# indrajeetadityaroy9/vit-inductive-bias-distillation

Hardware: AMD Instinct MI355X
Metric: distillation images/sec (BASD loss fwd+bwd+grad all-reduce), DeiT-S<-ResNet-50 @ bs256/GPU (higher is better)
Workload: dtype f32; 1 GPU; cfg2 DeiT-S<-ResNet-50 224x224; per_gpu_batch=256, global_batch=256, input_dtype=float32, layout=strided (CLS-sliced / channel-major views), backward=True, grad_allreduce_bytes=88202672, grad_allreduce=none at world size 1 (bucket packed, nothing to exchange), rank_readback=auto, readback_deferred_steps=1756, selector=basd_selector_chain mode 0, parallelism=dp1

## Files before the change

include/basd_hip.h:

```cpp
#ifndef BASD_HIP_H
#define BASD_HIP_H

#include <stdint.h>

#ifdef __cplusplus
extern "C" {
#endif

#ifndef __HIP_PLATFORM_AMD__
typedef struct ihipStream_t* hipStream_t;
#endif

#define BASD_OK 0
#define BASD_EINVAL (-1)
#define BASD_EUNSUPPORTED (-2)
#define BASD_DTYPE_F32 0
#define BASD_DTYPE_BF16 1
#define BASD_DTYPE_U8 2


int basd_gemm_nt(const void* a, int a_dtype, long a_sb, long a_sn, long a_sd, int a_rows_per_batch,
                 long a_batch_stride, const float* b, long ldb, long b_batch_stride, int M, int N, int K, int batch,
                 float* c, long ldc, long c_batch_stride, float scale, const float* bias, float beta,
                 float* colsum_part, float* col_mean, hipStream_t stream);
// ... 8 lines not shown
int basd_colmean_parts(int rows);

int basd_colmean(const void* x, int dtype, long sb, long sn, long sd, int rows_per_batch, long batch_stride,
                 int rows, int cols, int batch, int parts, float* partial, float* mean, hipStream_t stream);

int basd_gemm_tuning(int split_bf16);
int basd_gemm_tuning_get(void);

int basd_colmean_multi(const void* const* x_ptrs, int dtype, long sb, long sn, long sd, int rows_per_batch, int rows,
                       int cols, int n_mats, int parts, float* partial, float* means, int vec_ok,
                       hipStream_t stream);

int basd_syrk_splits(int krows, int cols, int n_mats);

int basd_syrk_multi(const void* const* x_ptrs, int dtype, long sb, long sn, long sd, int rows_per_batch, int krows,
                    int cols, int n_mats, const float* means, const float* scales, int splits, float* slabs,
                    float* out, long out_stride, int vec_ok, const float* fold, int fold_parts, int fold_from,
                    hipStream_t stream);


int basd_jacobi_workspace_ints(int batch, int max_sweeps);
int basd_jacobi_max_rows(void);
int basd_jacobi_plain4_fits(int n);

int basd_jacobi_tuning(int lanes_per_pair);
int basd_jacobi_ordering(int odd_even);

int basd_jacobi_onesided(float* W, long batch_stride, int rows_dot, int rows_tot, int n, int batch,
                         const int* n_arr, float* colnorm, int colnorm_stride, int max_sweeps, float tol_cos,
                         int* flags, int* sweeps_out, hipStream_t stream);

long basd_jacobi_twopass_workspace_bytes(int n, int batch, int max_sweeps);
int basd_jacobi_stacked_twopass(float* W, long batch_stride, int n, int batch, float* colnorm, int colnorm_stride,
                                int max_sweeps, float tol_cos, void* workspace, int* sweeps_out, hipStream_t stream);

int basd_sort_extract(const float* W, long batch_stride, int rows, int rows_tot, int n, int batch,
                      const float* colnorm, int colnorm_stride, float* vals_desc, float* vecs, int kmax,
                      hipStream_t stream);


long basd_tridiag_workspace_bytes(int n, int batch);

int basd_tridiag(float* a, long a_batch_stride, int n, int batch, float* d, float* e, float* tau, float* vh,
                 void* work, hipStream_t stream);

int basd_tridiag_ranked(float* a, long a_batch_stride, int n, int batch, float* d, float* e, float* tau, float* vh,
                        void* work, int rank_count, double factor, int cap, int* rank_out, int* host_mirror,
                        void* mid_event ,
                        hipStream_t stream);

int basd_tridiag_tuning(int members, int pad, int lag, int threads, int tail, int reset);

int basd_tridiag_eigenvalues(const float* d, const float* e, int n, int batch, float* vals_desc, hipStream_t stream);

int basd_tridiag_apply_q(const float* tau, const float* vh, int n, int k, int batch, const float* x, float* out,
                         int k_stride, int transpose, hipStream_t stream);

int basd_tridiag_shifted_solve(const float* d, const float* e, const float* shifts, int shift_stride, int n, int k,
                               int batch, const float* rhs, float* x, hipStream_t stream);

int basd_tridiag_mp_rank(const float* d, const float* e, int n, int batch, double factor, int cap, int* rank_out,
                         float* thr_out, const int* status, int* host_mirror, hipStream_t stream);

int basd_tridiag_eigenvectors(const float* d, const float* e, const float* tau, const float* vh,
                              const float* vals_desc, int n, int k, int batch, float* z, float* vecs, int k_stride,
                              hipStream_t stream);


int basd_mp_rank(const float* vals_desc, int n, int batch, double factor, int cap, int* rank_out, float* thr_out,
                 hipStream_t stream);

int basd_grassmann_distance(const float* colnorm, int stride, const int* k_arr, const float* sw, int sw_stride,
                            const int* sw_index, int items, float* d_out, float* theta_out, hipStream_t stream);

int basd_grassmann_distance_padded(const float* colnorm, int stride, int n_valid, const int* k_arr, const float* sw,
                                   int sw_stride, const int* sw_index, int items, float* d_out, hipStream_t stream);

int basd_sqrt_clamp(const float* in, float* out, long count, hipStream_t stream);

int basd_gram_finish(const float* c, const float* zbar, int n, int batch, long m_rows, float* out_u, float* out_c,
                     hipStream_t stream);

int basd_selector_tail(const float* t_d, const float* t_e, const float* t_tau, const float* t_vh, const float* t_vals,
                       const float* s_d, const float* s_e, const float* s_tau, const float* s_vh, const float* s_vals,
                       int d_s, int E, int L, int kmax, const int* ranks, const float* proj_s_t, float* z_s,
                       float* v_s, float* z_t, float* u_t, float* u_rot, float* sw, float* cos, int* k_arr,
                       const int* sw_index, float* sigma, int* flags, float* d_out, hipStream_t stream);

int basd_tridiag_mp_rank_rank1(const float* d, const float* e, const float* w, int n, int batch, double rho,
                               double factor, int cap, int* rank_out, const int* status, int* host_mirror,
                               hipStream_t stream);

int basd_tridiag_ranked_gated(float* a, long a_batch_stride, int n, int batch, float* d, float* e, float* tau, float* vh,
                              void* work, int rank_count, double factor, int cap, int* rank_out, int* host_mirror,
                              const unsigned* go_flag, unsigned go_value, int go_budget, hipStream_t stream);
int basd_flag_set(unsigned* flag, unsigned value, hipStream_t stream);

typedef struct BasdSelectorChain {
    const void* const* teacher_host_ptrs;
    long t_dtype, t_sb, t_sn, t_sd;
    const void* const* student_ptrs;
    long s_dtype, s_sb, s_sn, s_sd, s_vec_ok;
    const float* proj_t;
    const float* proj_s_t;
    long E, L, B, n_s, n_t, d_s, d_t;
    double mp_factor;
// ... 326 lines not shown
```

vit-inductive-bias-distillation_amd/basd_amd/_lib.py:

```python
from __future__ import annotations

import ctypes as C
import os
import threading

_HERE = os.path.dirname(os.path.abspath(__file__))
LIB_PATH = os.path.join(_HERE, "libbasd_hip.so")

vp, i32, i64, f32, f64 = C.c_void_p, C.c_int, C.c_long, C.c_float, C.c_double

SIGNATURES = {
    "basd_gemm_nt": [vp, i32, i64, i64, i64, i32, i64, vp, i64, i64, i32, i32, i32, i32, vp, i64, i64, f32, vp, f32,
                     vp, vp, vp],
    "basd_gemm_tn_splits": [i32],
    "basd_gemm_tn": [vp, vp, i32, i64, i64, i64, i64, i64, i64, i64, i64, i32, i32, i32, i32, i32, vp, vp, i32, vp,
                     vp, i64, i64, f32, vp],
    "basd_colmean_parts": [i32],
    "basd_colmean": [vp, i32, i64, i64, i64, i32, i64, i32, i32, i32, i32, vp, vp, vp],
    "basd_colmean_multi": [vp, i32, i64, i64, i64, i32, i32, i32, i32, i32, vp, vp, i32, vp],
    "basd_syrk_splits": [i32, i32, i32],
    "basd_syrk_multi": [vp, i32, i64, i64, i64, i32, i32, i32, i32, vp, vp, i32, vp, vp, i64, i32, vp, i32, i32, vp],
    "basd_jacobi_workspace_ints": [i32, i32],
    "basd_jacobi_max_rows": [],
    "basd_jacobi_twopass_workspace_bytes": [i32, i32, i32],
    "basd_jacobi_stacked_twopass": [vp, i64, i32, i32, vp, i32, i32, f32, vp, vp, vp],
    "basd_jacobi_tuning": [i32],
    "basd_jacobi_ordering": [i32],
    "basd_gemm_tuning": [i32],
    "basd_gemm_tuning_get": [],
    "basd_jacobi_onesided": [vp, i64, i32, i32, i32, i32, vp, vp, i32, i32, f32, vp, vp, vp],
    "basd_sort_extract": [vp, i64, i32, i32, i32, i32, vp, i32, vp, vp, i32, vp],
    "basd_tridiag_workspace_bytes": [i32, i32],
    "basd_tridiag_tuning": [i32, i32, i32, i32, i32, i32],
    "basd_tridiag": [vp, i64, i32, i32, vp, vp, vp, vp, vp, vp],
    "basd_tridiag_ranked": [vp, i64, i32, i32, vp, vp, vp, vp, vp, i32, f64, i32, vp, vp, vp, vp],
    "basd_tridiag_ranked_gated": [vp, i64, i32, i32, vp, vp, vp, vp, vp, i32, f64, i32, vp, vp, vp, C.c_uint, i32, vp],
    "basd_flag_set": [vp, C.c_uint, vp],
    "basd_scale_unless_one": [vp, i64, vp, vp, vp],
    "basd_event_create": [vp],
    "basd_event_destroy": [vp],
    "basd_stream_wait_event": [vp, vp],
    "basd_tridiag_eigenvalues": [vp, vp, i32, i32, vp, vp],
    "basd_tridiag_apply_q": [vp, vp, i32, i32, i32, vp, vp, i32, i32, vp],
    "basd_tridiag_shifted_solve": [vp, vp, vp, i32, i32, i32, i32, vp, vp, vp],
    "basd_tridiag_mp_rank": [vp, vp, i32, i32, f64, i32, vp, vp, vp, vp, vp],
    "basd_tridiag_mp_rank_rank1": [vp, vp, vp, i32, i32, f64, f64, i32, vp, vp, vp, vp],
    "basd_tridiag_eigenvectors": [vp, vp, vp, vp, vp, i32, i32, i32, vp, vp, i32, vp],
    "basd_mp_rank": [vp, i32, i32, f64, i32, vp, vp, vp],
    "basd_grassmann_distance": [vp, i32, vp, vp, i32, vp, i32, vp, vp, vp],
    "basd_grassmann_distance_padded": [vp, i32, i32, vp, vp, i32, vp, i32, vp, vp],
    "basd_selector_tail": [vp] * 10 + [i32, i32, i32, i32] + [vp] * 14 + [vp],
    "basd_sqrt_clamp": [vp, vp, i64, vp],
    "basd_gram_finish": [vp, vp, i32, i32, i64, vp, vp, vp],
    "basd_cross_entropy": [vp, i32, i64, i32, i32, vp, vp, i64, f32, i64, vp, vp, vp],
    "basd_token_weights": [vp, i32, vp, i32, i64, i64, i64, i64, i32, i32, i32, i32, i32, i32, i32, vp, vp, vp, vp,
                           vp, vp, vp, vp, vp, vp],
    "basd_student_project": [vp, i32, i64, i64, i32, i32, i32, i32, vp, vp, vp, vp, vp, vp, vp, vp, vp, vp],
    "basd_teacher_center": [vp, i32, vp, i32, i64, i64, i64, i32, i32, i32, vp, vp, vp, vp, vp, vp, vp],
    "basd_teacher_center_multi": [vp, i32, vp, i32, i32, i64, i64, i64, i32, i32, i32, vp, vp, vp, vp, vp, vp, vp],
    "basd_teacher_center_stream_scratch_floats": [i32, i32, i32, i32],
    "basd_teacher_center_stream": [vp, i32, vp, i32, i32, i64, i64, i64, i32, i32, i32, vp, vp, vp, vp, vp, vp, vp, vp],
    "basd_gram_f64": [vp, i64, i32, i32, i32, vp, i64, vp],
    "basd_gram_f64_split": [vp, i64, i32, i32, i32, i32, vp, vp, vp],
    "basd_chol_f64": [vp, i64, i32, i32, vp, i64, vp],
    "basd_stack_product": [vp, vp, i64, i32, i32, i32, vp, i64, vp],
    "basd_procrustes_finalize": [vp, i64, vp, i32, i32, i32, i32, vp, i64, vp, vp, vp, vp, vp, i32, vp, vp, vp, vp,
                                 vp, vp],
    "basd_student_project_multi": [vp, i32, i64, i64, i32, i32, i32, i32, i32, i32, vp, i64, vp, vp, vp, vp, vp, vp,
                                   vp, vp, vp],
    "basd_student_grad_multi": [vp, i32, i64, i64, i32, i32, i32, i32, i32, vp, i64, vp, vp, vp, vp, vp, vp, f32, vp,
                                vp, vp, vp],
    "basd_student_grad_fused": [vp, i32, i64, i64, i32, i32, i32, i32, i32, i32, vp, i64, vp, vp, vp, vp, vp, vp, vp,
                                f32, vp, vp],
    "basd_procrustes_forward_fused": [vp, vp],
    "basd_procrustes_tuning": [i32],
    "basd_jacobi_plain4_fits": [i32],
    "basd_stack_product_t": [vp, vp, i64, i32, i32, i32, vp, i64, vp],
    "basd_kprime_from_transposed": [vp, i64, vp, i32, i32, vp, i64, i32, vp, i64, vp, vp],
    "basd_procrustes_finish_transposed": [vp, i64, vp, i32, i32, i32, i32, vp, i64, vp, vp, vp, vp, vp, i32, vp, vp, vp,
                                          vp, vp, i64, i32, vp, vp],
    "basd_procrustes_finish_tuning": [i32],
    "basd_ustack_stash": [vp, i64, i32, i32, vp, i64, vp],
    "basd_ustack_from_transposed": [vp, i64, vp, i32, i32, vp, i64, vp, i64, vp, i32, vp, vp],
    "basd_resample_tokens": [vp, i32, i64, i64, i64, i32, i32, i32, i32, vp, vp, vp, vp, vp],
    "basd_resample_tokens_adjoint": [vp, i32, i32, i32, i32, vp, vp, vp, vp, vp, vp, vp],
    "basd_teacher_factor": [vp, i64, vp, i32, i32, i32, vp, vp, i64, vp, vp, vp, vp, vp, vp, vp, vp, vp],
    "basd_teacher_factor_tiled": [vp, i64, vp, i32, i32, i32, vp, vp, i64, vp, vp, vp, vp, vp, vp, vp, vp, vp, vp],
    "basd_mix_grad_tokens": [vp, vp, i32, i32, i64, i64, i64, i32, i32, i32, i32, vp, vp, vp, vp, vp],
    "basd_mix_grad_tokens_scratch_floats": [i32, i32, i32, i32],
    "basd_mix_grad_tokens_onepass": [vp, vp, i32, i32, i64, i64, i64, i32, i32, i32, i32, vp, vp, vp, vp, vp, vp],
    "basd_token_weight_bwd": [vp, vp, i32, i32, i32, i32, vp, vp, vp, vp, vp, vp, i32, i32, i64, i64, i64, i64, i32,
                              i32, i32, vp, vp, vp],
    "basd_build_angle_stack": [vp, i32, vp, i32, vp, vp],
    "basd_grassmann_distance_bwd": [vp, vp, i32, vp, vp, i32, vp, vp, i32, vp, vp],
    "basd_eigvec_k2": [vp, vp, i32, i32, i32, vp, vp],
# ... 117 lines not shown
```

vit-inductive-bias-distillation_amd/csrc/chain.hip:

```cpp
#include "basd_common.h"
#include "../../include/basd_hip.h"
#include <stdlib.h>

namespace basd {

__global__ void __launch_bounds__(256) chain_sw_kernel(const float* __restrict__ vals, int n, int kmax,
                                                       float* __restrict__ sw) {
    const int l = blockIdx.x;
    for (int i = threadIdx.x; i < kmax; i += 256) sw[(long)l * kmax + i] = sqrtf(fmaxf(vals[(long)l * n + i], 0.f));
}

__global__ void chain_k_arr_kernel(const int* __restrict__ ranks, int L, int items, int kmax, int* __restrict__ k_arr) {
    const int i = blockIdx.x * blockDim.x + threadIdx.x;
    if (i < items) {
        int k = ranks[i % L];
        k = k < 1 ? 1 : k;
        k_arr[i] = k > kmax ? kmax : k;
    }
}

constexpr int CERT_BLOCKS = 32;
__global__ void __launch_bounds__(256) rank_certificate_kernel(const float* __restrict__ grams, const float* __restrict__ zbar,
                                                               int n, int L, double factor, double* __restrict__ scratch,
                                                               int* __restrict__ host_flag) {
// ... 90 lines not shown
    } while (0)
#define BASD_MARK(ev, stream)                                         \
    do {                                                              \
        if (ev) BASD_HIP(hipEventRecord((hipEvent_t)(ev), (stream))); \
    } while (0)

extern "C" {

int basd_event_record(void* ev, hipStream_t stream) {
    BASD_CHECK_ARG(ev);
    BASD_HIP(hipEventRecord((hipEvent_t)ev, stream));
    return BASD_OK;
}
int basd_event_synchronize(void* ev) {
    BASD_CHECK_ARG(ev);
    BASD_HIP(hipEventSynchronize((hipEvent_t)ev));
    return BASD_OK;
}
int basd_stream_create_priority(void** out, int level) {
    BASD_CHECK_ARG(out && level >= -1 && level <= 1);
    int least = 0, greatest = 0;
    BASD_HIP(hipDeviceGetStreamPriorityRange(&least, &greatest));
    const int prio = level < 0 ? greatest : (level > 0 ? least : 0);
    BASD_HIP(hipStreamCreateWithPriority((hipStream_t*)out, hipStreamNonBlocking, prio));
    return BASD_OK;
}

int basd_event_create_timed(void** out) {
    BASD_CHECK_ARG(out);
    BASD_HIP(hipEventCreateWithFlags((hipEvent_t*)out, hipEventDefault));
    return BASD_OK;
}
int basd_event_elapsed_ms(void* from, void* to, float* ms_out) {
    BASD_CHECK_ARG(from && to && ms_out);
    BASD_HIP(hipEventElapsedTime(ms_out, (hipEvent_t)from, (hipEvent_t)to));
    return BASD_OK;
}

int basd_selector_chain_tail(const BasdSelectorChain* a, int kmax, int exact_k) {
    BASD_CHECK_ARG(a && a->d && a->vals && a->zv && a->vecs && a->u_rot && a->sw && a->cos && a->sigma && a->d_out &&
                   a->k_arr && a->sw_index && a->jflags && a->ranks && a->proj_s_t);
    const int E = (int)a->E, L = (int)a->L, n = (int)a->d_s;
    BASD_CHECK_ARG(E > 0 && L > 0 && kmax > 0 && kmax <= n && kmax <= (int)a->kmax_cap);
    if (!exact_k && !basd_jacobi_lds_square_fits(kmax) && !(kmax >= 96 && basd_jacobi_plain4_fits(kmax))) return BASD_EUNSUPPORTED;
    hipStream_t st = a->tail_stream;
    BASD_HIP(hipStreamWaitEvent(st, (hipEvent_t)a->ev_ranks, 0));
    if (a->mode != 0 && a->mode != 4) BASD_HIP(hipStreamWaitEvent(st, (hipEvent_t)a->ev_student, 0));
    const long nn = (long)n * n, kn = (long)kmax * n, kk = (long)kmax * kmax;
    const float* dz = a->d + (long)L * n;
    const float* ez = a->e + (long)L * n;
    const float* tz = a->tau + (long)L * n;
    const float* vz = a->vh + (long)L * nn;
    float* lam = a->vals + (long)L * n;
    BASD_TRY(basd_tridiag_eigenvalues(dz, ez, n, L + E, lam, st));
    BASD_MARK(a->tm_spec, st);
    BASD_TRY(basd_tridiag_eigenvectors(dz, ez, tz, vz, lam, n, kmax, L + E, a->zv, a->vecs, kmax, st));
    basd::chain_sw_kernel<<<L, 256, 0, st>>>(lam, n, kmax, a->sw);
    const float* u_t = a->vecs;
    const float* v_s = a->vecs + (long)L * kn;
    BASD_TRY(basd_gemm_nt(u_t, BASD_DTYPE_F32, 0, n, 1, 1 << 30, 0, a->proj_s_t, n, 0, L * kmax, n, n, 1, a->u_rot, n,
                          (long)L * kn, 1.f, nullptr, 0.f, nullptr, nullptr, st));
    if (L == 1) {
        BASD_TRY(basd_gemm_nt(v_s, BASD_DTYPE_F32, 0, n, 1, 1 << 30, kn, a->u_rot, n, 0, kmax, kmax, n, E, a->cos, kmax,
                              kk, 1.f, nullptr, 0.f, nullptr, nullptr, st));
    } else {
        for (int e = 0; e < E; ++e)
            BASD_TRY(basd_gemm_nt(v_s + e * kn, BASD_DTYPE_F32, 0, n, 1, 1 << 30, 0, a->u_rot, n, kn, kmax, kmax, n, L,
                                  a->cos + (long)e * L * kk, kmax, kk, 1.f, nullptr, 0.f, nullptr, nullptr, st));
    }
    const int items = E * L;
    basd::chain_k_arr_kernel<<<(items + 255) / 256, 256, 0, st>>>(a->ranks, L, items, kmax, a->k_arr);
    if (!exact_k && kmax >= 96 && basd_jacobi_plain4_fits(kmax)) {
        basd::chain_mask_cos_kernel<<<items, 256, 0, st>>>(a->cos, kmax, a->k_arr);
        BASD_TRY(basd_jacobi_onesided(a->cos, kk, kmax, kmax, kmax, items, nullptr, a->sigma, kmax, 20, 0.f, a->jflags,
                                      nullptr, st));
        BASD_TRY(basd_grassmann_distance_padded(a->sigma, kmax, kmax, a->k_arr, a->sw, kmax, a->sw_index, items, a->d_out,
                                                st));
    } else {
        BASD_TRY(basd_jacobi_onesided(a->cos, kk, kmax, kmax, kmax, items, exact_k ? nullptr : a->k_arr, a->sigma, kmax, 20,
                                      0.f, a->jflags, nullptr, st));
        BASD_TRY(basd_grassmann_distance(a->sigma, kmax, a->k_arr, a->sw, kmax, a->sw_index, items, a->d_out, nullptr, st));
    }
    BASD_HIP(hipEventRecord((hipEvent_t)a->ev_tail, st));
    return BASD_OK;
}

int basd_debug_fill_lds(unsigned pattern, hipStream_t stream) {
    const int bytes = 80 * 1024;
    (void)hipFuncSetAttribute((const void*)basd::debug_fill_lds_kernel, hipFuncAttributeMaxDynamicSharedMemorySize, bytes);
    basd::debug_fill_lds_kernel<<<4096, 256, bytes, stream>>>(pattern, bytes / 4);
    BASD_RETURN_LAST();
}

long basd_rank_certificate_scratch_bytes(int batch) { return batch > 0 ? 32L * batch + 8 : 0; }

int basd_rank_certificate(const float* grams, const float* zbar, int n, int batch, double factor, double* scratch,
                          int* flag, hipStream_t stream) {
    BASD_CHECK_ARG(grams && flag && scratch && n > 2 && batch > 0 && batch <= 65535 && factor > 0.0);
    basd::rank_certificate_kernel<<<dim3(basd::CERT_BLOCKS, batch), 256, 0, stream>>>(grams, zbar, n, batch, factor, scratch,
                                                                                     flag);
    BASD_RETURN_LAST();
}

int basd_selector_chain(const BasdSelectorChain* a) {
    BASD_CHECK_ARG(a && a->teacher_host_ptrs && a->student_ptrs && a->proj_t && a->z && a->z_sums && a->z_ptrs &&
                   a->z_means && a->t_slabs && a->s_partial && a->s_means && a->s_slabs && a->grams && a->d && a->e &&
                   a->tau && a->vh && a->tri_work && a->ranks && a->ev_fork && a->ev_student && a->ev_ranks && a->ev_tail);
// ... 99 lines not shown
```

vit-inductive-bias-distillation_amd/csrc/fused.hip:

```cpp
#include "basd_common.h"
#include "../../include/basd_hip.h"

namespace basd {

__global__ void __launch_bounds__(256) uwso_combine_kernel(const float* __restrict__ ce, const float* __restrict__ loss_b,
                                                           int E, int B, float* __restrict__ out) {
    constexpr int CH = 32;
    __shared__ double red[CH][4];
    const int tid = threadIdx.x;
    double geo_sum = 0.;
    for (int e0 = 0; e0 < E; e0 += CH) {
        const int ne = E - e0 < CH ? E - e0 : CH;
        for (int e = 0; e < ne; ++e) {
            double acc = 0.;
            for (int b = tid; b < B; b += 256) acc += (double)loss_b[(long)(e0 + e) * B + b];
            for (int m = 32; m > 0; m >>= 1) acc += __shfl_xor(acc, m, 64);
            if ((tid & 63) == 0) red[e][tid >> 6] = acc;
        }
        __syncthreads();
        if (tid == 0)
            for (int e = 0; e < ne; ++e) {
                const float layer = (float)(((red[e][0] + red[e][1]) + (red[e][2] + red[e][3])) / (double)B);
                out[4 + E + e0 + e] = layer;
                geo_sum += (double)layer;
            }
        __syncthreads();
    }
    if (tid == 0) {
        const float c = ce[0], geo = (float)(geo_sum / (double)E);
        const float eps = 1.1920929e-7f;
        const float i0 = 1.f / fmaxf(c, eps), i1 = 1.f / fmaxf(geo, eps);
        const float w0 = i0 / (i0 + i1), w1 = i1 / (i0 + i1);
        out[0] = w0;
        out[1] = w1;
        out[2] = w0 * c + w1 * geo;
        out[3] = geo;
        for (int e = 0; e < E; ++e) out[4 + e] = w1 / (float)E;
    }
}

__global__ void __launch_bounds__(256) scale_unless_one_kernel(float* __restrict__ x, long count4, long count,
                                                               const float* __restrict__ num,
                                                               const float* __restrict__ den) {
    const float f = den ? num[0] / den[0] : num[0];
    if (f == 1.f) return;
    const long i = (long)blockIdx.x * 256 + threadIdx.x;
    if (i < count4) {
        float4 v = ((float4*)x)[i];
        v.x *= f; v.y *= f; v.z *= f; v.w *= f;
        ((float4*)x)[i] = v;
    }
    if (blockIdx.x == 0 && threadIdx.x < (int)(count - 4 * count4)) x[4 * count4 + threadIdx.x] *= f;
}

}

extern "C" {

int basd_scale_unless_one(float* x, long count, const float* num, const float* den, hipStream_t stream) {
    BASD_CHECK_ARG(x && num && count > 0 && ((uintptr_t)x & 15) == 0);
    const long count4 = count / 4;
    basd::scale_unless_one_kernel<<<(unsigned)((count4 + 255) / 256 + (count4 == 0)), 256, 0, stream>>>(x, count4, count, num, den);
    BASD_RETURN_LAST();
}

static int procrustes_tail(const BasdProcrustesArgs* a, const float* grad_layers, int E, int B, int n_s, int n, int d_s,
                           int EB, long nn, long om_stride, hipStream_t st) {
    int rc;
#define BASD_TRY(call)            \
    do {                          \
        rc = (call);              \
        if (rc != BASD_OK) return rc; \
    } while (0)
    if (a->uw_ce) {
        BASD_CHECK_ARG(a->uw_out != nullptr);
        basd::uwso_combine_kernel<<<1, 256, 0, st>>>(a->uw_ce, a->loss_b, E, B, a->uw_out);
        grad_layers = a->uw_out + 4;
    }
    if (a->dx) {
        BASD_CHECK_ARG(a->k_prime && a->h && grad_layers);
        rc = basd_student_grad_fused(a->student_ptrs, (int)a->s_dtype, a->s_sb, a->s_sn, E, B, n_s, n, d_s,
                                     (int)a->s_aligned, a->omega, om_stride, a->mu_s, a->k_prime, a->a_prime, a->tap0,
                                     a->tap1, a->lam, grad_layers, 2.0f / (float)B, a->dx, st);
        if (rc != BASD_EUNSUPPORTED) return rc;
        BASD_TRY(basd_gemm_tn(a->k_prime, a->a_prime, BASD_DTYPE_F32, 0, n, 1, nn, 0, d_s, 1, (long)n * d_s, 1 << 30, n,
                              n, d_s, EB, nullptr, nullptr, 1, nullptr, a->h, d_s, (long)n * d_s, 1.f, st));
        BASD_TRY(basd_student_grad_multi(a->student_ptrs, (int)a->s_dtype, a->s_sb, a->s_sn, E, B, n_s, n, d_s, a->omega,
                                         om_stride, a->mu_s, a->h, a->tap0, a->tap1, a->lam, grad_layers,
                                         2.0f / (float)B, a->dx, nullptr, nullptr, st));
    }
#undef BASD_TRY
    return BASD_OK;
}

static int g_transposed_cores = 1;
int basd_procrustes_tuning(int transposed_cores) {
    if (transposed_cores >= 0) g_transposed_cores = transposed_cores > 2 ? 2 : transposed_cores;
    return BASD_OK;
}
static int g_finish_fused = 1;
int basd_procrustes_finish_tuning(int fused) {
    const int prev = g_finish_fused;
    if (fused >= 0) g_finish_fused = fused ? 1 : 0;
    return prev;
}

int basd_procrustes_forward_fused(const BasdProcrustesArgs* a, hipStream_t st) {
    BASD_CHECK_ARG(a && a->student_ptrs && a->tok_ptrs && a->attn_ptrs && a->mix);
    const int E = (int)a->E, L = (int)a->L, G = (int)a->G, B = (int)a->B, n_s = (int)a->n_s, n_t = (int)a->n_t;
    const int d_s = (int)a->d_s, d_t = (int)a->d_t, H = (int)a->H, A = (int)a->A, n_a = (int)a->n_a, n = (int)a->n;
    const float* grad_layers_in = a->grad_layers;
    BASD_CHECK_ARG(E > 0 && L > 0 && (G == 1 || G == E) && B > 0 && n == (n_s < n_t ? n_s : n_t));
    int rc;
#define BASD_TRY(call)            \
    do {                          \
// ... 112 lines not shown
```

vit-inductive-bias-distillation_amd/csrc/tridiag.hip:

```cpp
#include "basd_common.h"
#include <stdlib.h>
#include <atomic>

namespace basd {

__device__ __forceinline__ void lds_barrier() { asm volatile("s_waitcnt lgkmcnt(0)\n\ts_barrier" ::: "memory"); }

__device__ __forceinline__ float block_sum_lds(float v, float* scratch, int nw) {
    v = wave_sum(v);
    if ((threadIdx.x & 63) == 0) scratch[threadIdx.x >> 6] = v;
    lds_barrier();
    float r = 0.f;
    for (int i = 0; i < nw; ++i) r += scratch[i];
    return r;
}

typedef unsigned tri_u32x4 __attribute__((ext_vector_type(4)));
typedef float tri_f32x4 __attribute__((ext_vector_type(4)));
__device__ __forceinline__ void granule_store(uint4* p, float a, float b, unsigned tag) {
    const tri_u32x4 x = {__float_as_uint(a), __float_as_uint(b), tag, __float_as_uint(a) ^ __float_as_uint(b) ^ tag};
    asm volatile("global_store_dwordx4 %0, %1, off sc1\n\ts_nop 1" ::"v"(p), "v"(x) : "memory");
}
__device__ __forceinline__ tri_u32x4 granule_load(const uint4* p) {
    tri_u32x4 x;
// ... 889 lines not shown
        }
        __builtin_amdgcn_fence(__ATOMIC_ACQUIRE, "agent");
    }
    const long long wall0 = wall_clock64(), clk0 = clock64();
    __shared__ __attribute__((aligned(16))) float optab[WAVES][CH][24];
    __shared__ __attribute__((aligned(16))) float colf[64][20];
    __shared__ __attribute__((aligned(16))) float part[WAVES][64][8];
    __shared__ __attribute__((aligned(16))) float yrows[WAVES][PK_RPW];
    __shared__ float cap[PK_NMAX];
    __shared__ float dloc[PK_NMAX], eloc[PK_NMAX], tloc[PK_NMAX];
    const int z = blockIdx.x, tid = threadIdx.x, lane = tid & 63;
    const int wave = __builtin_amdgcn_readfirstlane(tid >> 6);
    const int pl = pk_pi(lane);
    float* Az = A + (long)z * a_batch_stride;
    float* Vz = Vh + (long)z * n * n;
    const float* const optab_w = &optab[wave][0][0];
    float* const yrow_q = &yrows[wave][0] + 2 * (((lane >> 5) & 1) | ((lane >> 3) & 2));
    float* const pub = &optab[lane >> 3][0][0] + (lane & 7);
    const float* const ugather = &optab[lane & 7][0][0] + 16 + (lane >> 3);

    tri_f2 A2[84];
#pragma unroll
    for (int P = 0; P < PK_PAIRS; ++P) {
        const int ra = wave + 16 * P, rb = ra + 8;
#pragma unroll
        for (int k = P >> 2; k < CH; ++k) {
            const int c = pl + 64 * k;
            float xa = 0.f, xb = 0.f;
            if (c < n) {
                if (ra < n && c >= ra) xa = Az[(long)ra * n + c] * (c == ra ? 0.5f : 1.f);
                if (rb < n && c >= rb) xb = Az[(long)rb * n + c] * (c == rb ? 0.5f : 1.f);
            }
            A2[pk_idx(P, k)] = tri_f2{xa, xb};
        }
    }
    tri_f2 MK2[4];
#pragma unroll
    for (int q = 0; q < 4; ++q) {
        const int ta = wave + 16 * q, tb = ta + 8;
        MK2[q] = tri_f2{pl > ta ? 1.f : (pl == ta ? 0.5f : 0.f), pl > tb ? 1.f : (pl == tb ? 0.5f : 0.f)};
    }

    float tau = 0.f;
    auto pick = [&](const float (&x)[CH], int c) {
        const int l = pk_pi(c & 63);
        return uniform_select6(lane_bcast(x[0], l), lane_bcast(x[1], l), lane_bcast(x[2], l), lane_bcast(x[3], l),
                               lane_bcast(x[4], l), lane_bcast(x[5], l), c >> 6);
    };
    auto next_reflector = [&](int jl, bool last, const float (&cn)[CH], const float (&uc)[CH], const float (&wn)[CH],
                              float dnew) {
        const int r0 = jl + 1;
        float part2 = 0.f;
#pragma unroll
        for (int k = 0; k < CH; ++k) part2 = (pl + 64 * k > r0) ? fmaf(cn[k], cn[k], part2) : part2;
        const float alpha = pick(cn, r0 < PK_NMAX ? r0 : PK_NMAX - 1);
        const float xn2 = wave_sum(part2);
        const bool live = !last && xn2 > 0.f;
        const float beta = live ? -copysignf(__builtin_amdgcn_sqrtf(fmaf(alpha, alpha, xn2)), alpha) : (last ? 0.f : alpha);
        tau = live ? (beta - alpha) * __builtin_amdgcn_rcpf(beta) : 0.f;
        const float scal = live ? __builtin_amdgcn_rcpf(alpha - beta) : 0.f;
        float un[CH];
#pragma unroll
        for (int k = 0; k < CH; ++k) {
            const int c = pl + 64 * k;
            un[k] = last ? 0.f : (c < r0 ? 0.f : (c == r0 ? 1.f : cn[k] * scal));
            pub[24 * k] = uc[k];
            pub[24 * k + 8] = wn[k];
            pub[24 * k + 16] = un[k];
        }
        tri_f32x4* cf = (tri_f32x4*)&colf[lane][0];
        cf[0] = tri_f32x4{un[0], un[1], un[2], un[3]};
        cf[1] = tri_f32x4{un[4], un[5], uc[0], uc[1]};
        cf[2] = tri_f32x4{uc[2], uc[3], uc[4], uc[5]};
        cf[3] = tri_f32x4{wn[0], wn[1], wn[2], wn[3]};
        cf[4] = tri_f32x4{wn[4], wn[5], 0.f, 0.f};
        if (lane == 0) {
            dloc[jl] = dnew;
            eloc[jl] = beta;
            tloc[jl] = tau;
        }
    };
    auto store_reflector = [&](int jl) {
        const int k = wave - 1;
        if (k >= 0 && k < CH && lane + 64 * k < n)
            Vz[(long)jl * n + lane + 64 * k] = ugather[24 * k];
    };
    if (wave == 0) {
        float cn[CH], zero[CH];
#pragma unroll
        for (int k = 0; k < CH; ++k) {
            cn[k] = A2[pk_idx(0, k)].x * ((k == 0 && pl == 0) ? 2.f : 1.f);
            zero[k] = 0.f;
        }
        next_reflector(0, n <= 1, cn, zero, zero, pick(cn, 0));
    }
    lds_barrier();
    store_reflector(0);

    for (int jl = 0; jl < n - 1; ++jl) {
        const int r0 = jl + 1;
        PK_STAMP(0);
        tri_f2 NV[3], NW[3], UC[3], acc2[CH];
        {
            const tri_f32x4* cf = (const tri_f32x4*)&colf[lane][0];
            const tri_f32x4 c0 = cf[0], c1 = cf[1], c2 = cf[2], c3 = cf[3], c4 = cf[4];
            UC[0] = tri_f2{c0.x, c0.y}; UC[1] = tri_f2{c0.z, c0.w}; UC[2] = tri_f2{c1.x, c1.y};
            NV[0] = tri_f2{c1.z, c1.w}; NV[1] = tri_f2{c2.x, c2.y}; NV[2] = tri_f2{c2.z, c2.w};
            NW[0] = tri_f2{c3.x, c3.y}; NW[1] = tri_f2{c3.z, c3.w}; NW[2] = tri_f2{c4.x, c4.y};
#pragma unroll
            for (int k = 0; k < CH; ++k) acc2[k] = tri_f2{0.f, 0.f};
        }
        {
            const int i0 = r0 > wave ? (r0 - wave + 7) >> 3 : 0;
            switch (i0 >> 3) {
                PK_BATCH(0)
                PK_BATCH(1)
                PK_BATCH(2)
                PK_BATCH(3)
                PK_BATCH(4)
                PK_BATCH(5)
                default: break;
            }
        }
        if (wave == (r0 & (WAVES - 1))) {
            const int i0r = r0 >> 3, half = i0r & 1;
            const float capfix = pl == (r0 & 63) ? 2.f : 1.f;
            switch (i0r >> 1) {
                PK_CAP(0) PK_CAP(1) PK_CAP(2) PK_CAP(3) PK_CAP(4) PK_CAP(5) PK_CAP(6) PK_CAP(7)
                PK_CAP(8) PK_CAP(9) PK_CAP(10) PK_CAP(11) PK_CAP(12) PK_CAP(13) PK_CAP(14) PK_CAP(15)
                PK_CAP(16) PK_CAP(17) PK_CAP(18) PK_CAP(19) PK_CAP(20) PK_CAP(21) PK_CAP(22) PK_CAP(23)
                default: break;
            }
        }
        {
            tri_f32x4* pp = (tri_f32x4*)&part[wave][lane][0];
            pp[0] = tri_f32x4{acc2[0].x + acc2[0].y, acc2[1].x + acc2[1].y, acc2[2].x + acc2[2].y, acc2[3].x + acc2[3].y};
            pp[1] = tri_f32x4{acc2[4].x + acc2[4].y, acc2[5].x + acc2[5].y, 0.f, 0.f};
        }
        PK_STAMP(1);
        lds_barrier();
        PK_STAMP(2);
        if (wave == 0) {
            float uc[CH];
            uc[0] = UC[0].x; uc[1] = UC[0].y; uc[2] = UC[1].x; uc[3] = UC[1].y; uc[4] = UC[2].x; uc[5] = UC[2].y;
            const float cap_r0 = cap[(r0 >> 6) * 64 + pk_pi(r0 & 63)];
            tri_f2 sc2[3] = {{0.f, 0.f}, {0.f, 0.f}, {0.f, 0.f}};
#pragma unroll
            for (int w = 0; w < WAVES; ++w) {
                const tri_f32x4* pp = (const tri_f32x4*)&part[w][lane][0];
                const tri_f32x4 p0 = pp[0];
                const tri_f2 p1 = *(const tri_f2*)&pp[1];
                sc2[0] = pk_add(sc2[0], tri_f2{p0.x, p0.y});
                sc2[1] = pk_add(sc2[1], tri_f2{p0.z, p0.w});
                sc2[2] = pk_add(sc2[2], p1);
            }
            tri_f2 pc2[3], capc2[3];
            const tri_f2 tau2 = {tau, tau};
#pragma unroll
            for (int q = 0; q < 3; ++q) {
                const tri_f2 y2 = {yrows[lane >> 3][16 * q + (lane & 7)], yrows[lane >> 3][16 * q + 8 + (lane & 7)]};
                pc2[q] = pk_mul(tau2, pk_add(sc2[q], y2));
                capc2[q] = tri_f2{cap[128 * q + lane], cap[128 * q + 64 + lane]};
            }
            PK_STAMP(3);
            tri_f2 dot2 = {0.f, 0.f};
#pragma unroll
            for (int q = 0; q < 3; ++q) pk_fma(dot2, pc2[q], UC[q]);
            float pc[CH];
            pc[0] = pc2[0].x; pc[1] = pc2[0].y; pc[2] = pc2[1].x; pc[3] = pc2[1].y; pc[4] = pc2[2].x; pc[5] = pc2[2].y;
            const float p_r0 = pick(pc, r0);
            const float gamma = -0.5f * tau * wave_sum(dot2.x + dot2.y);
            const float w0 = p_r0 + gamma;
            float wn[CH], cn[CH];
            {
                const tri_f2 g2 = {gamma, gamma}, w02 = {w0, w0};
#pragma unroll
                for (int q = 0; q < 3; ++q) {
                    tri_f2 wn2 = pc2[q];
                    pk_fma(wn2, g2, UC[q]);
                    tri_f2 t2_ = wn2;
                    pk_fma(t2_, UC[q], w02);
                    const tri_f2 cn2 = pk_add(capc2[q], tri_f2{-t2_.x, -t2_.y});
                    wn[2 * q] = wn2.x; wn[2 * q + 1] = wn2.y;
                    cn[2 * q] = cn2.x; cn[2 * q + 1] = cn2.y;
                }
            }
            PK_STAMP(4);
            next_reflector(jl + 1, jl + 1 >= n - 1, cn, uc, wn, cap_r0 - fmaf(1.f, w0, w0));
            PK_STAMP(5);
        }
        lds_barrier();
        PK_STAMP(6);
        store_reflector(jl + 1);
    }
    lds_barrier();
    {
        float* dz = d + (long)z * n;
        float* ez = e + (long)z * n;
        float* tz = tau_out + (long)z * n;
        for (int c = tid; c < n; c += 64 * WAVES) {
            dz[c] = dloc[c];
            ez[c] = eloc[c];
            tz[c] = tloc[c];
        }
    }
    if (clocks && z == 0 && tid == 0 && rk.status) {
        int* st = const_cast<int*>(rk.status);
        st[6] = (int)(wall_clock64() - wall0);
        st[7] = (int)((clock64() - clk0) >> 4);
    }
    if (rk.rank_out && z < rk.count) {
        __syncthreads();
        mp_rank_block(dloc, eloc, n, z, rk, nullptr);
    }
}
#undef PK_CHUNK
// ... 704 lines not shown
            tridiag_packed_kernel<<<batch, 64 * PK_WAVES, 0, stream>>>(a, a_batch_stride, n, d, e, tau, vh, in_tail, g_pk_clocks, go_flag, go_value, go_budget);
        else if (g_tuning.tail == 2)
            tridiag_tail_kernel<16, 16, 4><<<batch, 1024, 0, stream>>>(a, a_batch_stride, n, j_stop, j_stop > 0 ? pend : nullptr, d, e, tau, vh, in_tail);
        else
            tridiag_tail2_kernel<<<batch, 512, 0, stream>>>(a, a_batch_stride, n, j_stop, j_stop > 0 ? pend : nullptr, d, e, tau, vh, in_tail);
    }
    if (rk.rank_out && !fused_rank)
        tridiag_mp_rank_kernel<<<rk.count, 1024, 0, stream>>>(d, e, n, rk.factor, rk.cap, rk.rank_out, nullptr, rk.host_mirror ? err : nullptr, rk.host_mirror);
    BASD_RETURN_LAST();
}

int basd_tridiag(float* a, long a_batch_stride, int n, int batch, float* d, float* e, float* tau, float* vh,
                 void* work, hipStream_t stream) {
    return tridiag_impl(a, a_batch_stride, n, batch, d, e, tau, vh, work, MpRankOut{nullptr, nullptr, nullptr, 0., 0, 0}, stream);
}

int basd_tridiag_ranked(float* a, long a_batch_stride, int n, int batch, float* d, float* e, float* tau, float* vh,
                        void* work, int rank_count, double factor, int cap, int* rank_out, int* host_mirror,
                        void* mid_event, hipStream_t stream) {
    BASD_CHECK_ARG(rank_out && rank_count > 0 && rank_count <= batch);
    if (n > 8192) return BASD_EUNSUPPORTED;
    return tridiag_impl(a, a_batch_stride, n, batch, d, e, tau, vh, work,
                        MpRankOut{rank_out, host_mirror, nullptr, factor, cap, rank_count}, stream,
                        (hipEvent_t)mid_event);
}

int basd_tridiag_ranked_gated(float* a, long a_batch_stride, int n, int batch, float* d, float* e, float* tau, float* vh,
                              void* work, int rank_count, double factor, int cap, int* rank_out, int* host_mirror,
                              const unsigned* go_flag, unsigned go_value, int go_budget, hipStream_t stream) {
    BASD_CHECK_ARG(rank_out && rank_count > 0 && rank_count <= batch && go_flag && go_value != 0 && go_budget > 0);
    return tridiag_impl(a, a_batch_stride, n, batch, d, e, tau, vh, work,
                        MpRankOut{rank_out, host_mirror, nullptr, factor, cap, rank_count}, stream, nullptr, go_flag,
                        go_value, go_budget);
}

namespace basd {
__global__ void flag_set_kernel(unsigned* flag, unsigned value) {
    __hip_atomic_store(flag, value, __ATOMIC_RELEASE, __HIP_MEMORY_SCOPE_AGENT);
}
}
int basd_flag_set(unsigned* flag, unsigned value, hipStream_t stream) {
    BASD_CHECK_ARG(flag);
    basd::flag_set_kernel<<<1, 1, 0, stream>>>(flag, value);
    BASD_RETURN_LAST();
}

int basd_tridiag_eigenvalues(const float* d, const float* e, int n, int batch, float* vals_desc, hipStream_t stream) {
    BASD_CHECK_ARG(d && e && vals_desc && n > 0 && batch > 0);
    if (n > 8192) return BASD_EUNSUPPORTED;
    sturm_bisect_kernel<<<dim3((n + 63) / 64, batch), 1024, 0, stream>>>(d, e, n, vals_desc);
    BASD_RETURN_LAST();
}

int basd_tridiag_apply_q(const float* tau, const float* vh, int n, int k, int batch, const float* x, float* out,
                         int k_stride, int transpose, hipStream_t stream) {
    BASD_CHECK_ARG(tau && vh && x && out && n > 1 && k > 0 && batch > 0 && k_stride >= k);
    const dim3 grid((k + 3) / 4, batch);
#define BASD_APPLY_Q(E)                                                                                          \
    do {                                                                                                          \
        if (transpose) backtransform_kernel<E, true><<<grid, 256, 0, stream>>>(vh, tau, n, k, x, out, k_stride);  \
        else backtransform_kernel<E, false><<<grid, 256, 0, stream>>>(vh, tau, n, k, x, out, k_stride);           \
    } while (0)
    if (n <= 192) BASD_APPLY_Q(3);
    else if (n <= 384) BASD_APPLY_Q(6);
    else if (n <= 768) BASD_APPLY_Q(12);
    else if (n <= 1024) BASD_APPLY_Q(16);
    else return BASD_EUNSUPPORTED;
#undef BASD_APPLY_Q
    BASD_RETURN_LAST();
}

int basd_tridiag_shifted_solve(const float* d, const float* e, const float* shifts, int shift_stride, int n, int k,
                               int batch, const float* rhs, float* x, hipStream_t stream) {
    BASD_CHECK_ARG(d && e && shifts && rhs && x && n > 1 && k > 0 && batch > 0 && shift_stride >= k);
    int vpw = (int)((144 * 1024) / (6 * sizeof(float) * (size_t)n));
    if (vpw > 64) vpw = 64;
    if (vpw < 1) return BASD_EUNSUPPORTED;
    const size_t lds_a = sizeof(float) * 6 * (size_t)n * vpw;
    if (lds_a > 48 * 1024)
        (void)hipFuncSetAttribute((const void*)tridiag_shifted_solve_kernel, hipFuncAttributeMaxDynamicSharedMemorySize, (int)lds_a);
    tridiag_shifted_solve_kernel<<<dim3((k + vpw - 1) / vpw, batch), 64, lds_a, stream>>>(d, e, shifts, shift_stride, n, k, vpw, rhs, x);
    BASD_RETURN_LAST();
}

int basd_tridiag_mp_rank(const float* d, const float* e, int n, int batch, double factor, int cap, int* rank_out,
                         float* thr_out, const int* status, int* host_mirror, hipStream_t stream) {
    BASD_CHECK_ARG(d && e && rank_out && n > 0 && batch > 0);
    if (n > 8192) return BASD_EUNSUPPORTED;
    tridiag_mp_rank_kernel<<<batch, 1024, 0, stream>>>(d, e, n, factor, cap, rank_out, thr_out, status, host_mirror);
    BASD_RETURN_LAST();
}

int basd_tridiag_mp_rank_rank1(const float* d, const float* e, const float* w, int n, int batch, double rho,
                               double factor, int cap, int* rank_out, const int* status, int* host_mirror,
                               hipStream_t stream) {
    BASD_CHECK_ARG(d && e && w && rank_out && n > 0 && batch > 0 && rho > 0.);
    if (n > 8192) return BASD_EUNSUPPORTED;
    tridiag_mp_rank1_kernel<<<batch, 1024, 0, stream>>>(d, e, w, n, rho, factor, cap, rank_out, status, host_mirror);
    BASD_RETURN_LAST();
}

#ifdef BASD_TAIL_DBG
int basd_debug_tail_stamps(long long* host_out) {
    return (int)hipMemcpyFromSymbol(host_out, HIP_SYMBOL(basd::g_tail_dbg), sizeof(long long) * 2 * 8 * 2 * 1024);
}
#endif
// ... 31 lines not shown
```

Before: 170,900 images/s.

## Compute only leading tridiagonal eigenvalues and tidy several tridiag/scale kernels

Adds a leading-eigenvalue entry point that launches the Sturm bisection kernel over only ceil(k/64) blocks instead of ceil(n/64), and the chain calls it with kmax, so eigenvalues beyond kmax are never computed. Separately, the scale-unless-one kernel becomes grid-stride with its grid capped at 1024 blocks. Inside the tridiagonal reduction, the y/cap loads are hoisted ahead of the partial-sum reduction, and the index comparisons and reflector store addressing are rewritten. The eigenvalue trim assumes the bisection kernel derives eigenvalue indices from blockIdx, and that later code (mp_rank, chain_sw) reads only the first kmax values.

Result: faster. 175,300 images/s, median of 6 (+2.6%).

```diff
diff --git a/include/basd_hip.h b/include/basd_hip.h
--- a/include/basd_hip.h
+++ b/include/basd_hip.h
@@ -84,6 +84,9 @@
 int basd_tridiag_tuning(int members, int pad, int lag, int threads, int tail, int reset);
 
 int basd_tridiag_eigenvalues(const float* d, const float* e, int n, int batch, float* vals_desc, hipStream_t stream);
+
+int basd_tridiag_eigenvalues_leading(const float* d, const float* e, int n, int k, int batch, float* vals_desc,
+                                     hipStream_t stream);
 
 int basd_tridiag_apply_q(const float* tau, const float* vh, int n, int k, int batch, const float* x, float* out,
                          int k_stride, int transpose, hipStream_t stream);
diff --git a/vit-inductive-bias-distillation_amd/basd_amd/_lib.py b/vit-inductive-bias-distillation_amd/basd_amd/_lib.py
--- a/vit-inductive-bias-distillation_amd/basd_amd/_lib.py
+++ b/vit-inductive-bias-distillation_amd/basd_amd/_lib.py
@@ -41,6 +41,7 @@
     "basd_event_destroy": [vp],
     "basd_stream_wait_event": [vp, vp],
     "basd_tridiag_eigenvalues": [vp, vp, i32, i32, vp, vp],
+    "basd_tridiag_eigenvalues_leading": [vp, vp, i32, i32, i32, vp, vp],
     "basd_tridiag_apply_q": [vp, vp, i32, i32, i32, vp, vp, i32, i32, vp],
     "basd_tridiag_shifted_solve": [vp, vp, vp, i32, i32, i32, i32, vp, vp, vp],
     "basd_tridiag_mp_rank": [vp, vp, i32, i32, f64, i32, vp, vp, vp, vp, vp],
diff --git a/vit-inductive-bias-distillation_amd/csrc/chain.hip b/vit-inductive-bias-distillation_amd/csrc/chain.hip
--- a/vit-inductive-bias-distillation_amd/csrc/chain.hip
+++ b/vit-inductive-bias-distillation_amd/csrc/chain.hip
@@ -166,7 +166,7 @@
     const float* tz = a->tau + (long)L * n;
     const float* vz = a->vh + (long)L * nn;
     float* lam = a->vals + (long)L * n;
-    BASD_TRY(basd_tridiag_eigenvalues(dz, ez, n, L + E, lam, st));
+    BASD_TRY(basd_tridiag_eigenvalues_leading(dz, ez, n, kmax, L + E, lam, st));
     BASD_MARK(a->tm_spec, st);
     BASD_TRY(basd_tridiag_eigenvectors(dz, ez, tz, vz, lam, n, kmax, L + E, a->zv, a->vecs, kmax, st));
     basd::chain_sw_kernel<<<L, 256, 0, st>>>(lam, n, kmax, a->sw);
diff --git a/vit-inductive-bias-distillation_amd/csrc/fused.hip b/vit-inductive-bias-distillation_amd/csrc/fused.hip
--- a/vit-inductive-bias-distillation_amd/csrc/fused.hip
+++ b/vit-inductive-bias-distillation_amd/csrc/fused.hip
@@ -44,8 +44,7 @@
                                                                const float* __restrict__ den) {
     const float f = den ? num[0] / den[0] : num[0];
     if (f == 1.f) return;
-    const long i = (long)blockIdx.x * 256 + threadIdx.x;
-    if (i < count4) {
+    for (long i = (long)blockIdx.x * 256 + threadIdx.x; i < count4; i += (long)gridDim.x * 256) {
         float4 v = ((float4*)x)[i];
         v.x *= f; v.y *= f; v.z *= f; v.w *= f;
         ((float4*)x)[i] = v;
@@ -60,7 +59,8 @@
 int basd_scale_unless_one(float* x, long count, const float* num, const float* den, hipStream_t stream) {
     BASD_CHECK_ARG(x && num && count > 0 && ((uintptr_t)x & 15) == 0);
     const long count4 = count / 4;
-    basd::scale_unless_one_kernel<<<(unsigned)((count4 + 255) / 256 + (count4 == 0)), 256, 0, stream>>>(x, count4, count, num, den);
+    const long groups = (count4 + 255) / 256 + (count4 == 0);
+    basd::scale_unless_one_kernel<<<(unsigned)(groups < 1024 ? groups : 1024), 256, 0, stream>>>(x, count4, count, num, den);
     BASD_RETURN_LAST();
 }
 
diff --git a/vit-inductive-bias-distillation_amd/csrc/tridiag.hip b/vit-inductive-bias-distillation_amd/csrc/tridiag.hip
--- a/vit-inductive-bias-distillation_amd/csrc/tridiag.hip
+++ b/vit-inductive-bias-distillation_amd/csrc/tridiag.hip
@@ -965,7 +965,7 @@
         const int r0 = jl + 1;
         float part2 = 0.f;
 #pragma unroll
-        for (int k = 0; k < CH; ++k) part2 = (pl + 64 * k > r0) ? fmaf(cn[k], cn[k], part2) : part2;
+        for (int k = 0; k < CH; ++k) part2 = (pl > r0 - 64 * k) ? fmaf(cn[k], cn[k], part2) : part2;
         const float alpha = pick(cn, r0 < PK_NMAX ? r0 : PK_NMAX - 1);
         const float xn2 = wave_sum(part2);
         const bool live = !last && xn2 > 0.f;
@@ -975,8 +975,8 @@
         float un[CH];
 #pragma unroll
         for (int k = 0; k < CH; ++k) {
-            const int c = pl + 64 * k;
-            un[k] = last ? 0.f : (c < r0 ? 0.f : (c == r0 ? 1.f : cn[k] * scal));
+            const int rk_ = r0 - 64 * k;
+            un[k] = last ? 0.f : (pl < rk_ ? 0.f : (pl == rk_ ? 1.f : cn[k] * scal));
             pub[24 * k] = uc[k];
             pub[24 * k + 8] = wn[k];
             pub[24 * k + 16] = un[k];
@@ -995,8 +995,10 @@
     };
     auto store_reflector = [&](int jl) {
         const int k = wave - 1;
-        if (k >= 0 && k < CH && lane + 64 * k < n)
-            Vz[(long)jl * n + lane + 64 * k] = ugather[24 * k];
+        if (k >= 0 && k < CH && lane + 64 * k < n) {
+            float* const vrow = Vz + ((long)jl * n + 64 * k);
+            vrow[(unsigned)lane] = ugather[24 * k];
+        }
     };
     if (wave == 0) {
         float cn[CH], zero[CH];
@@ -1057,6 +1059,12 @@
             float uc[CH];
             uc[0] = UC[0].x; uc[1] = UC[0].y; uc[2] = UC[1].x; uc[3] = UC[1].y; uc[4] = UC[2].x; uc[5] = UC[2].y;
             const float cap_r0 = cap[(r0 >> 6) * 64 + pk_pi(r0 & 63)];
+            tri_f2 y2[3], capc2[3];
+#pragma unroll
+            for (int q = 0; q < 3; ++q) {
+                y2[q] = tri_f2{yrows[lane >> 3][16 * q + (lane & 7)], yrows[lane >> 3][16 * q + 8 + (lane & 7)]};
+                capc2[q] = tri_f2{cap[128 * q + lane], cap[128 * q + 64 + lane]};
+            }
             tri_f2 sc2[3] = {{0.f, 0.f}, {0.f, 0.f}, {0.f, 0.f}};
 #pragma unroll
             for (int w = 0; w < WAVES; ++w) {
@@ -1067,14 +1075,10 @@
                 sc2[1] = pk_add(sc2[1], tri_f2{p0.z, p0.w});
                 sc2[2] = pk_add(sc2[2], p1);
             }
-            tri_f2 pc2[3], capc2[3];
+            tri_f2 pc2[3];
             const tri_f2 tau2 = {tau, tau};
 #pragma unroll
-            for (int q = 0; q < 3; ++q) {
-                const tri_f2 y2 = {yrows[lane >> 3][16 * q + (lane & 7)], yrows[lane >> 3][16 * q + 8 + (lane & 7)]};
-                pc2[q] = pk_mul(tau2, pk_add(sc2[q], y2));
-                capc2[q] = tri_f2{cap[128 * q + lane], cap[128 * q + 64 + lane]};
-            }
+            for (int q = 0; q < 3; ++q) pc2[q] = pk_mul(tau2, pk_add(sc2[q], y2[q]));
             PK_STAMP(3);
             tri_f2 dot2 = {0.f, 0.f};
 #pragma unroll
@@ -1885,6 +1889,15 @@
     BASD_RETURN_LAST();
 }
 
+int basd_tridiag_eigenvalues_leading(const float* d, const float* e, int n, int k, int batch, float* vals_desc,
+                                     hipStream_t stream) {
+    BASD_CHECK_ARG(d && e && vals_desc && n > 0 && k > 0 && batch > 0);
+    if (n > 8192) return BASD_EUNSUPPORTED;
+    if (k > n) k = n;
+    sturm_bisect_kernel<<<dim3((k + 63) / 64, batch), 1024, 0, stream>>>(d, e, n, vals_desc);
+    BASD_RETURN_LAST();
+}
+
 int basd_tridiag_apply_q(const float* tau, const float* vh, int n, int k, int batch, const float* x, float* out,
                          int k_stride, int transpose, hipStream_t stream) {
     BASD_CHECK_ARG(tau && vh && x && out && n > 1 && k > 0 && batch > 0 && k_stride >= k);
```
